# ywz978020607/MASIC

Hardware: AMD Instinct MI355X
Metric: stereo pairs/sec (enc+dec) (higher is better)
Workload: dtype bf16; 1 GPU; HSIC(N=128,M=192,K=5) eval forward (enc+dec both views), 8x3x512x512 stereo pairs per GPU (BASELINE.json configs[1] shape), inputs resident in HBM (the graph's static input buffers); the device homography of batch k+1 is handed over with batch k (one-batch look-ahead of a loader): its device->host read, the float32 host chain and the upload of the sampling matrices are done every step, under the r; pairs_per_gpu=8, height=512, width=512, parallelism=dp1 (pairs sharded, no data-path collective)

## Files before the change

masic_amd/csrc/conv.hip:

```cpp
#include "common.h"
#include "conv_geom.h"

namespace {
struct ConvCfg {
    int direct;
    int wvm;
    int wm;
    int wn;
    int buf_sz;
    int vec4;
    int bf16;
    int pf;
    int KC, KClog;
    int TW, TWlog, SR, TH;
    int Cin_pad, Cout_pad;
    int PH, PW, PWp, PSZ;
    int max_taps;
    size_t lds_bytes;
};

int ilog2(int v) { int l = 0; while ((1 << l) < v) ++l; return l; }

ConvCfg choose_cfg(const masic_conv_desc_t& d, const ConvGeom* g, int nphase) {
    ConvCfg c{};
// ... 537 lines not shown
            st.y = apply_act(acc[ph][1][o] + bv, a.act);
            *reinterpret_cast<float2*>(yo + (size_t)(2 * r + ph) * a.Wo + 2 * c) = st;
        }
    }
}

__global__ void pack_deconv4_kernel(const float* __restrict__ w, float* __restrict__ wp, int Cin, int Cin_pad, int Cout) {
    const int i = blockIdx.x * blockDim.x + threadIdx.x;
    if (i >= Cin_pad * 100) return;
    const int ci = i / 100, rem = i - ci * 100, tap = rem >> 2, o = rem & 3;
    wp[i] = (ci < Cin && o < Cout) ? w[((size_t)ci * Cout + o) * 25 + tap] : 0.0f;
}


typedef __bf16 bf16x8 __attribute__((ext_vector_type(8)));
constexpr int MAXP = 6;

__device__ __forceinline__ unsigned pack_bf16x2(float lo, float hi) {
    typedef __bf16 bf16x2 __attribute__((ext_vector_type(2)));
    bf16x2 v;
    v[0] = (__bf16)lo;
    v[1] = (__bf16)hi;
    return __builtin_bit_cast(unsigned, v);
}

template <int WVM, int WM, int WN, int INOP, bool PF>
__global__ __launch_bounds__(256, 2) void conv_igemm_bf16(const IgemmArgs a, const unsigned short* __restrict__ wpk) {
    constexpr int BM = 32 * WM * WVM;
    constexpr int DEPTH = WM * WN >= 8 ? 4 : (WM * WN >= 2 ? 8 : 16);
    extern __shared__ __attribute__((aligned(16))) float lds[];
    unsigned short* patch = reinterpret_cast<unsigned short*>(lds);
    const int KCP = a.KC + 8;
    const int tid = threadIdx.x, lane = tid & 63;
    const int wave = __builtin_amdgcn_readfirstlane(tid >> 6);
    const int wm = wave % WVM, wn = wave / WVM;
    const int j = lane & 31, h = lane >> 5;

    const int phase = blockIdx.x % a.nphase, tile = blockIdx.x / a.nphase;
    const ConvGeom g = make_geom(a.q, phase);
    const int tw_i = tile % a.tiles_w, th_i = tile / a.tiles_w;
    const int m0 = blockIdx.y * BM;
    const int b = blockIdx.z;
    const int r0 = th_i * a.TH, c0 = tw_i * a.TW;
    const int ih0 = r0 * g.is + g.dh_min, iw0 = c0 * g.is + g.dw_min;

    const int NP = a.PH * a.PW;
    const size_t plane = (size_t)a.Hi * a.Wi;
    const float* xb = a.x + ((size_t)b * a.in_ctot + a.in_coff) * plane;
    auto pixel_offset = [&](int p) {
        const int pr = p / a.PW, pc = p - pr * a.PW;
        const int ih = ih0 + pr, iw = iw0 + pc;
        return (ih >= 0 && ih < a.Hi && iw >= 0 && iw < a.Wi) ? ih * a.Wi + iw : -1;
    };
    constexpr int NT = PF ? 4 : MAXP;
    int goff[NT], gch_t[PF ? 4 : 1], loff[PF ? 4 : 1];
    const int ngroups = a.KC >> 3;
#pragma unroll
    for (int i = 0; i < NT; ++i) {
        const int t = tid + 256 * i;
        if (PF) {
            const int gq = t / NP, p = t - gq * NP;
            goff[i] = gq >= ngroups ? -2 : pixel_offset(p);
            gch_t[i] = gq * 8;
            loff[i] = p * KCP + gq * 8;
        } else {
            goff[i] = t >= NP ? -2 : pixel_offset(t);
        }
    }

    const int jr = j >> a.TWlog, jc = j & (a.TW - 1);
    int lane_p[WN];
#pragma unroll
    for (int n = 0; n < WN; ++n) {
        const int r = (wn * WN + n) * a.SR + jr;
        lane_p[n] = ((r * g.is) * a.PW + jc * g.is) * KCP + 8 * h;
    }
    f32x16 acc[WM][WN];
#pragma unroll
    for (int m = 0; m < WM; ++m)
#pragma unroll
        for (int n = 0; n < WN; ++n)
#pragma unroll
            for (int e = 0; e < 16; ++e) acc[m][n][e] = 0.0f;

    const int ksteps = a.KC >> 4, kslog = ksteps >> 1;
    const int nsteps = g.ntaps * ksteps;
    const int tap0_off = ((g.dh0 - g.dh_min) * a.PW + (g.dw0 - g.dw_min)) * KCP;
    const int row_step = (g.dsh * a.PW - g.dsw * (g.ntw - 1)) * KCP;
    const int col_step = g.dsw * KCP;
    const int cin16 = a.Cin_pad >> 4;
    const size_t a_lane = ((size_t)m0 + wm * (32 * WM) + j) * 16 + 8 * h;
    const size_t a_tap_stride = (size_t)cin16 * a.Cout_pad * 16;
    const size_t a_c16_stride = (size_t)a.Cout_pad * 16;

    float pre[PF ? 4 : 1][8];
    auto load_tasks = [&](int cc) {
#pragma unroll
        for (int i = 0; i < (PF ? 4 : 1); ++i) {
#pragma unroll
            for (int c = 0; c < 8; ++c) {
                const int cg = cc + gch_t[i] + c;
                pre[i][c] = xb[(size_t)(cg < a.Cin ? cg : a.Cin - 1) * plane + (goff[i] >= 0 ? goff[i] : 0)];
            }
        }
    };
    auto store_tasks = [&](int cc) {
#pragma unroll
        for (int i = 0; i < (PF ? 4 : 1); ++i) {
            if (goff[i] == -2) continue;
            float v[8];
#pragma unroll
            for (int c = 0; c < 8; ++c)
                v[c] = (goff[i] >= 0 && cc + gch_t[i] + c < a.Cin) ? apply_inop(pre[i][c], INOP) : 0.0f;
            uint4 q;
            q.x = pack_bf16x2(v[0], v[1]); q.y = pack_bf16x2(v[2], v[3]);
            q.z = pack_bf16x2(v[4], v[5]); q.w = pack_bf16x2(v[6], v[7]);
            *reinterpret_cast<uint4*>(patch + loff[i]) = q;
        }
    };
    if (PF) load_tasks(0);

    for (int cc = 0; cc < a.Cin_pad; cc += a.KC) {
        if (PF) {
            store_tasks(cc);
        } else {
            for (int gch = 0; gch < a.KC; gch += 8) {
                float v[NT][8];
#pragma unroll
                for (int c = 0; c < 8; ++c) {
                    const int cg = cc + gch + c;
                    if (cg < a.Cin) {
                        const float* xc = xb + (size_t)cg * plane;
#pragma unroll
                        for (int i = 0; i < NT; ++i) {
                            const float t = xc[goff[i] >= 0 ? goff[i] : 0];
                            v[i][c] = goff[i] >= 0 ? t : 0.0f;
                        }
                    } else {
#pragma unroll
                        for (int i = 0; i < NT; ++i) v[i][c] = 0.0f;
                    }
                }
#pragma unroll
                for (int i = 0; i < NT; ++i) {
                    if (goff[i] == -2) continue;
                    uint4 q;
                    q.x = pack_bf16x2(apply_inop(v[i][0], INOP), apply_inop(v[i][1], INOP));
                    q.y = pack_bf16x2(apply_inop(v[i][2], INOP), apply_inop(v[i][3], INOP));
                    q.z = pack_bf16x2(apply_inop(v[i][4], INOP), apply_inop(v[i][5], INOP));
                    q.w = pack_bf16x2(apply_inop(v[i][6], INOP), apply_inop(v[i][7], INOP));
                    *reinterpret_cast<uint4*>(patch + (size_t)(tid + 256 * i) * KCP + gch) = q;
                }
            }
        }
        __syncthreads();
        if (PF && cc + a.KC < a.Cin_pad) load_tasks(cc + a.KC);
        const unsigned short* wa = wpk + (size_t)g.tap_base * a_tap_stride + (size_t)(cc >> 4) * a_c16_stride + a_lane;
        auto a_offset = [&](int st) { return (size_t)(st >> kslog) * a_tap_stride + (size_t)(st & (ksteps - 1)) * a_c16_stride; };
        uint4 ring[DEPTH][WM];
#pragma unroll
        for (int u = 0; u < DEPTH; ++u)
            if (u < nsteps) {
                const unsigned short* pa = wa + a_offset(u);
#pragma unroll
                for (int m = 0; m < WM; ++m) ring[u][m] = *reinterpret_cast<const uint4*>(pa + m * 32 * 16);
            }
        int sp = tap0_off, kk = 0, tb = 0;
        for (int st0 = 0; st0 < nsteps; st0 += DEPTH) {
#pragma unroll
            for (int u = 0; u < DEPTH; ++u) {
                const int st = st0 + u;
                if (st < nsteps) {
                    bf16x8 bfrag[WN], afr[WM];
#pragma unroll
                    for (int n = 0; n < WN; ++n)
                        bfrag[n] = __builtin_bit_cast(bf16x8, *reinterpret_cast<const uint4*>(patch + sp + lane_p[n] + kk * 16));
#pragma unroll
                    for (int m = 0; m < WM; ++m) afr[m] = __builtin_bit_cast(bf16x8, ring[u][m]);
                    if (st + DEPTH < nsteps) {
                        const unsigned short* pa = wa + a_offset(st + DEPTH);
#pragma unroll
                        for (int m = 0; m < WM; ++m) ring[u][m] = *reinterpret_cast<const uint4*>(pa + m * 32 * 16);
                    }
#pragma unroll
                    for (int m = 0; m < WM; ++m)
#pragma unroll
                        for (int n = 0; n < WN; ++n)
                            acc[m][n] = __builtin_amdgcn_mfma_f32_32x32x16_bf16(afr[m], bfrag[n], acc[m][n], 0, 0, 0);
                    if (++kk == ksteps) {
                        kk = 0;
                        if (++tb < g.ntw) sp += col_step;
                        else { tb = 0; sp += row_step; }
                    }
                }
            }
        }
        __syncthreads();
    }

    if (a.y16 != nullptr) {
        igemm_epilogue_f16k<WM, WN>(a, g, acc, b, m0 + wm * (32 * WM), r0, c0, wn, jr, jc, h);
        return;
    }
    igemm_epilogue<WM, WN>(a, g, acc, b, m0 + wm * (32 * WM), r0, c0, wn, jr, jc, h);
}


struct Conv5s1Args {
    const float* x; const float* bias; const float* gate; const float* res1; float* y;
    int Cin, H, W, in_ctot, in_coff, Cout, out_ctot, out_coff, act, tiles_w, gate_ctot, gate_c;
    const float* xb;
    int split;
    const float* gin_beta; const float* gin_gamma; int gin_inverse;
    const float* gout_beta; const float* gout_gamma; int gout_inverse;
    float beta_bound, gamma_bound, pedestal;
};

__device__ __forceinline__ void gdn3(float (&v)[3], const float* beta, const float* gamma, int inverse, float bb, float gb, float ped) {
    float sq[3], o[3];
#pragma unroll
    for (int k = 0; k < 3; ++k) sq[k] = __fmul_rn(v[k], v[k]);
#pragma unroll
    for (int i = 0; i < 3; ++i) {
        const float bv = fmaxf(beta[i], bb);
        float n = __fsub_rn(__fmul_rn(bv, bv), ped);
        float s = 0.0f;
#pragma unroll
        for (int k = 0; k < 3; ++k) {
            const float g = fmaxf(gamma[i * 3 + k], gb);
            s = fmaf(__fsub_rn(__fmul_rn(g, g), ped), sq[k], s);
        }
        n += s;
        const float r = sqrtf(n);
        o[i] = inverse ? v[i] * r : v[i] * (1.0f / r);
    }
#pragma unroll
    for (int i = 0; i < 3; ++i) v[i] = o[i];
}

template <int CO>
__global__ __launch_bounds__(256) void conv5s1_small(const Conv5s1Args a, const float* __restrict__ wpk) {
    constexpr int T = 16, LW = T + 4, PLANE = LW * LW, PSZ = 448;
    __shared__ __attribute__((aligned(16))) float lds[8 * PSZ];
    const int tid = threadIdx.x, lane = tid & 63;
    const int wave = __builtin_amdgcn_readfirstlane(tid >> 6);
    const int tx = tid & 15, ty = ((tid >> 4) & 3) * 4 + (tid >> 6);
    const int tile_x = blockIdx.x % a.tiles_w, tile_y = blockIdx.x / a.tiles_w;
    const int b = blockIdx.y;
    const int oy = tile_y * T + ty, ox = tile_x * T + tx;
    const size_t plane = (size_t)a.H * a.W;
    const float* xb = a.x + ((size_t)b * a.in_ctot + a.in_coff) * plane;
    const int split = a.xb != nullptr ? a.split : a.Cin;
    const float* xb2 = a.xb != nullptr ? a.xb + (size_t)b * (a.Cin - split) * plane : nullptr;
    for (int cg = wave; cg < a.Cin * 7; cg += 4) {
        const int ci = cg / 7, g = cg - ci * 7;
        const int e = g * 64 + lane;
        const int pr = e / LW, pc = e - pr * LW;
        const int ih = tile_y * T - 2 + pr, iw = tile_x * T - 2 + pc;
        const bool ok = e < PLANE && ih >= 0 && ih < a.H && iw >= 0 && iw < a.W;
        const float* src = ci < split ? xb + (size_t)ci * plane : xb2 + (size_t)(ci - split) * plane;
        if (e < PLANE) dma4(ok ? src + (size_t)ih * a.W + iw : g_zero_word, lds + ci * PSZ + g * 64);
    }
    __syncthreads();
    if (a.gin_beta != nullptr) {
        for (int e = tid; e < PLANE; e += 256) {
            float v[3] = {lds[e], lds[PSZ + e], lds[2 * PSZ + e]};
            gdn3(v, a.gin_beta, a.gin_gamma, a.gin_inverse, a.beta_bound, a.gamma_bound, a.pedestal);
            lds[e] = v[0]; lds[PSZ + e] = v[1]; lds[2 * PSZ + e] = v[2];
        }
        __syncthreads();
    }
    float acc[CO];
#pragma unroll
    for (int o = 0; o < CO; ++o) acc[o] = 0.0f;
    const float* base = lds + ty * LW + tx;
    for (int ci = 0; ci < a.Cin; ++ci) {
        const float* w = wpk + ci * 25 * CO;
        const float* pl = base + ci * PSZ;
#pragma unroll
        for (int kh = 0; kh < 5; ++kh)
#pragma unroll
            for (int kw = 0; kw < 5; ++kw) {
                const float xv = pl[kh * LW + kw];
#pragma unroll
                for (int o = 0; o < CO; ++o) acc[o] = fmaf(xv, w[(kh * 5 + kw) * CO + o], acc[o]);
            }
    }
    if (oy >= a.H || ox >= a.W) return;
    const size_t opix = (size_t)oy * a.W + ox;
    const float gv = a.gate ? a.gate[((size_t)b * a.gate_ctot + a.gate_c) * plane + opix] : 1.0f;
    if (a.gout_beta != nullptr) {
        float v[3] = {acc[0] + (a.bias ? a.bias[0] : 0.0f), acc[1] + (a.bias ? a.bias[1] : 0.0f), acc[2] + (a.bias ? a.bias[2] : 0.0f)};
        gdn3(v, a.gout_beta, a.gout_gamma, a.gout_inverse, a.beta_bound, a.gamma_bound, a.pedestal);
#pragma unroll
        for (int o = 0; o < 3; ++o) a.y[((size_t)b * a.out_ctot + a.out_coff + o) * plane + opix] = v[o];
        return;
    }
#pragma unroll
    for (int o = 0; o < CO; ++o) {
        if (o >= a.Cout) break;
        float v = apply_act(acc[o] + (a.bias ? a.bias[o] : 0.0f), a.act) * gv;
        if (a.res1) v += a.res1[((size_t)b * a.Cout + o) * plane + opix];
        a.y[((size_t)b * a.out_ctot + a.out_coff + o) * plane + opix] = v;
    }
}

__global__ void pack_conv5s1_kernel(const float* __restrict__ w, float* __restrict__ wp, int Cin, int Cout, int transposed, int CO) {
    const int i = blockIdx.x * blockDim.x + threadIdx.x;
    if (i >= Cin * 25 * CO) return;
    const int ci = i / (25 * CO), rem = i - ci * 25 * CO, tap = rem / CO, o = rem - tap * CO;
    float v = 0.0f;
    if (o < Cout) v = transposed ? w[((size_t)ci * Cout + o) * 25 + (24 - tap)] : w[((size_t)o * Cin + ci) * 25 + tap];
    wp[i] = v;
}


}

extern "C" size_t masic_conv_packed_bytes(const masic_conv_desc_t* d) {
    if (check_desc(d) != MASIC_OK) return 0;
    ConvGeom g[4];
    const int np = build_geoms(*d, g);
    const ConvCfg c = choose_cfg(*d, g, np);
    int taps = 0;
    for (int p = 0; p < np; ++p) taps += g[p].ntaps;
    if (c.direct == 2) return (size_t)c.Cin_pad * 100 * sizeof(float);
    if (c.direct == 3) return (size_t)c.Cin_pad * 25 * c.Cout_pad * sizeof(float);
    if (c.bf16) return (size_t)taps * c.Cin_pad * c.Cout_pad * sizeof(unsigned short);
    return (size_t)taps * c.Cin_pad * c.Cout_pad * sizeof(float);
}

extern "C" int masic_conv_variant(const masic_conv_desc_t* d, int* launches) {
    int rc = check_desc(d);
    if (rc != MASIC_OK) return rc;
    ConvGeom g[4];
    const int np = build_geoms(*d, g);
    const ConvCfg c = choose_cfg(*d, g, np);
    if (launches) *launches = 1;
    if (c.direct == 2) return 6;
    if (c.direct == 3) return 11;
    if (c.direct) return d->Cout <= 3 ? 0 : 1;
    if (c.bf16) return 10;
    if (c.wvm == 1) return c.wm == 1 ? 8 : 9;
    if (c.wm == 2) return c.wn == 4 ? 5 : 7;
    return c.wn == 4 ? 4 : (c.wn == 2 ? 3 : 2);
}

extern "C" int masic_conv_kernel_name(const masic_conv_desc_t* d, char* buf, size_t n) {
    int rc = check_desc(d);
    if (rc != MASIC_OK) return rc;
    MASIC_REQUIRE(buf && n > 0, MASIC_ERR_ARG, "conv_kernel_name: null buffer");
    ConvGeom g[4];
    const int np = build_geoms(*d, g);
    const ConvCfg c = choose_cfg(*d, g, np);
    if (c.direct == 2) snprintf(buf, n, "deconv5s2_small_cout");
    else if (c.direct == 3) snprintf(buf, n, "conv5s1_small");
    else if (c.direct) snprintf(buf, n, "conv_direct_f32<%d>", d->Cout <= 3 ? 3 : 8);
    else if (c.bf16) snprintf(buf, n, "conv_igemm_bf16<%d, %d, %d, %d, %s>", c.wvm, c.wm, c.wn, d->in_op, c.pf ? "true" : "false");
    else snprintf(buf, n, "conv_igemm_f32<%d, %d, %d, %d, %s>", c.wvm, c.wm, c.wn, d->in_op, c.vec4 ? "true" : "false");
    return MASIC_OK;
}

extern "C" int masic_conv_pack_weight(const float* w, void* w_packed, const masic_conv_desc_t* d, void* stream) {
    int rc = check_desc(d);
    if (rc != MASIC_OK) return rc;
    MASIC_REQUIRE(w && w_packed, MASIC_ERR_ARG, "conv_pack_weight: null pointer");
    ConvGeom g[4];
    const int np = build_geoms(*d, g);
    const ConvCfg c = choose_cfg(*d, g, np);
    if (c.direct == 2) {
        hipLaunchKernelGGL(pack_deconv4_kernel, dim3(ceil_div(c.Cin_pad * 100, 256)), dim3(256), 0, (hipStream_t)stream,
                           w, (float*)w_packed, d->Cin, c.Cin_pad, d->Cout);
        return masic_launch_status("conv_pack_weight");
    }
    if (c.direct == 3) {
        hipLaunchKernelGGL(pack_conv5s1_kernel, dim3(ceil_div(d->Cin * 25 * c.Cout_pad, 256)), dim3(256), 0, (hipStream_t)stream,
                           w, (float*)w_packed, d->Cin, d->Cout, d->transposed, c.Cout_pad);
        return masic_launch_status("conv_pack_weight");
    }
    PackArgs a{w, (float*)w_packed, d->Cin, d->Cout, d->KH, d->KW, c.Cin_pad, c.Cout_pad, d->transposed, {}};
    int max_taps = 0;
    for (int p = 0; p < np; ++p) {
        a.gs[p] = g[p];
        max_taps = max_taps > g[p].ntaps ? max_taps : g[p].ntaps;
    }
    const size_t total = (size_t)max_taps * c.Cin_pad * c.Cout_pad;
    int blocks = (int)((total + 255) / 256);
    if (blocks > 4096) blocks = 4096;
    if (c.bf16) hipLaunchKernelGGL(pack_weight_bf16_kernel, dim3(blocks, np), dim3(256), 0, (hipStream_t)stream, a, (unsigned short*)w_packed);
    else hipLaunchKernelGGL(pack_weight_kernel, dim3(blocks, np), dim3(256), 0, (hipStream_t)stream, a);
    return masic_launch_status("conv_pack_weight");
}

extern "C" int masic_conv2d_fwd_ex(const float* x, const void* w_packed, const float* bias, const float* gate,
                                   const float* res1, const float* res2, float* y, const masic_conv_desc_t* d, void* stream);

extern "C" int masic_conv2d_fwd(const float* x, const void* w_packed, const float* bias, const float* gate,
                                float* y, const masic_conv_desc_t* d, void* stream) {
    return masic_conv2d_fwd_ex(x, w_packed, bias, gate, nullptr, nullptr, y, d, stream);
}

namespace {
int conv2d_launch(const float* x, const void* w_packed, const float* bias, const float* gate,
                  const float* res1, const float* res2, float* y, void* y_f16k, const masic_conv_desc_t* d, void* stream);
}

extern "C" int masic_conv2d_fwd_ex(const float* x, const void* w_packed, const float* bias, const float* gate,
                                   const float* res1, const float* res2, float* y, const masic_conv_desc_t* d, void* stream) {
    MASIC_REQUIRE(y != nullptr, MASIC_ERR_ARG, "conv2d_fwd: null pointer");
    return conv2d_launch(x, w_packed, bias, gate, res1, res2, y, nullptr, d, stream);
}

extern "C" int masic_conv2d_f16k_out_supported(const masic_conv_desc_t* d) {
    if (check_desc(d) != MASIC_OK || d->prec != MASIC_PREC_BF16 || d->Cout % 32 != 0 || d->out_ctot % 16 != 0 || d->out_coff % 16 != 0) return 0;
    ConvGeom g[4];
    const int np = build_geoms(*d, g);
    const ConvCfg c = choose_cfg(*d, g, np);
    return !c.direct && c.bf16;
}

extern "C" int masic_conv2d_f16k_out_fwd(const float* x, const void* w_packed, const float* bias, void* y_f16k,
                                         const masic_conv_desc_t* d, void* stream) {
    MASIC_REQUIRE(y_f16k != nullptr && d != nullptr, MASIC_ERR_ARG, "conv2d_f16k_out_fwd: null pointer");
    MASIC_REQUIRE(masic_conv2d_f16k_out_supported(d), MASIC_ERR_UNSUPPORTED,
                  "conv2d_f16k_out_fwd: needs bf16 operands on the implicit-GEMM kernel, Cout % 32 == 0 and a 16-aligned output view");
    return conv2d_launch(x, w_packed, bias, nullptr, nullptr, nullptr, nullptr, y_f16k, d, stream);
}

namespace {
int conv2d_launch(const float* x, const void* w_packed, const float* bias, const float* gate,
                  const float* res1, const float* res2, float* y, void* y_f16k, const masic_conv_desc_t* d, void* stream) {
    int rc = check_desc(d);
    if (rc != MASIC_OK) return rc;
    MASIC_REQUIRE(d->prec != MASIC_PREC_FP8, MASIC_ERR_UNSUPPORTED, "conv2d_fwd: fp8 operands exist on the F8K entry points only (masic_conv_f8k_fwd)");
    MASIC_REQUIRE(x && w_packed && (y || y_f16k), MASIC_ERR_ARG, "conv2d_fwd: null pointer");
    ConvGeom g[4];
    const int np = build_geoms(*d, g);
    const ConvCfg c = choose_cfg(*d, g, np);
    MASIC_REQUIRE(y_f16k == nullptr || (!c.direct && c.bf16), MASIC_ERR_UNSUPPORTED, "conv2d_fwd: F16K output exists on conv_igemm_bf16 only");
    hipStream_t st = (hipStream_t)stream;
    const GeomParams q = geom_params(*d);
    if (g[0].Hp <= 0 || g[0].Wp <= 0) return MASIC_OK;
    if (c.direct == 2) {
        MASIC_REQUIRE(gate == nullptr && res1 == nullptr && res2 == nullptr, MASIC_ERR_UNSUPPORTED, "conv2d_fwd: gate/residual on the small-Cout deconv path");
        MASIC_REQUIRE(d->Wo % 2 == 0, MASIC_ERR_SHAPE, "conv2d_fwd: odd output width");
        Deconv4Args a{x, (const float*)w_packed, bias, y, d->Cin, c.Cin_pad, d->Hi, d->Wi, d->in_ctot, d->in_coff,
                      d->Cout, d->Ho, d->Wo, d->out_ctot, d->out_coff, d->act, ceil_div(d->Wi, 16)};
        hipLaunchKernelGGL(deconv5s2_small_cout, dim3(ceil_div(d->Wi, 16) * ceil_div(d->Hi, 16), d->B), dim3(256), 0, st, a,
                           (const float*)w_packed);
        return masic_launch_status("conv2d_fwd");
    }
    if (c.direct == 3) {
        MASIC_REQUIRE(res2 == nullptr, MASIC_ERR_UNSUPPORTED, "conv2d_fwd: two residuals on the small 5x5 path");
        Conv5s1Args a{x, bias, gate, res1, y, d->Cin, d->Hi, d->Wi, d->in_ctot, d->in_coff, d->Cout, d->out_ctot, d->out_coff,
                      d->act, ceil_div(d->Wi, 16), d->gate_ctot, d->gate_c, nullptr, 0, nullptr, nullptr, 0, nullptr, nullptr, 0, 0.0f, 0.0f, 0.0f};
        if (c.Cout_pad == 4) hipLaunchKernelGGL(conv5s1_small<4>, dim3(ceil_div(d->Wi, 16) * ceil_div(d->Hi, 16), d->B), dim3(256), 0, st, a,
                                                (const float*)w_packed);
        else hipLaunchKernelGGL(conv5s1_small<8>, dim3(ceil_div(d->Wi, 16) * ceil_div(d->Hi, 16), d->B), dim3(256), 0, st, a,
                                (const float*)w_packed);
        return masic_launch_status("conv2d_fwd");
    }
    if (c.direct) {
        DirectArgs a{x, (const float*)w_packed, bias, gate, res1, res2, y,
                     d->Cin, d->Hi, d->Wi, d->in_ctot, d->in_coff,
                     d->Cout, d->Ho, d->Wo, d->out_ctot, d->out_coff,
                     d->in_op, d->act, d->gate_ctot, d->gate_c, q, np};
        dim3 grid(ceil_div(g[0].Hp * g[0].Wp, 256) * np, d->B);
        if (d->Cout <= 3) hipLaunchKernelGGL(conv_direct_f32<3>, grid, dim3(256), 0, st, a);
        else hipLaunchKernelGGL(conv_direct_f32<8>, grid, dim3(256), 0, st, a);
        return masic_launch_status("conv2d_fwd");
    }
    {
        IgemmArgs a{x, (const float*)w_packed, bias, gate, res1, res2, y,
                    d->Cin, d->Hi, d->Wi, d->in_ctot, d->in_coff,
                    d->Cout, d->Ho, d->Wo, d->out_ctot, d->out_coff,
                    c.Cin_pad, c.Cout_pad, c.KC, c.KClog,
                    c.TW, c.TWlog, c.SR, c.TH, ceil_div(g[0].Wp, c.TW),
                    c.PH, c.PW, c.PWp, c.PSZ, c.buf_sz, c.vec4,
                    d->in_op, d->act, d->gate_ctot, d->gate_c, q, np, (unsigned short*)y_f16k};
        dim3 grid(ceil_div(g[0].Wp, c.TW) * ceil_div(g[0].Hp, c.TH) * np, c.Cout_pad / (32 * c.wm * c.wvm), d->B);
        if (c.bf16) {
#define BF16_LAUNCH(WV, WMV, WNV, OPV)                                                                                            \
    do {                                                                                                                          \
        if (c.pf) hipLaunchKernelGGL((conv_igemm_bf16<WV, WMV, WNV, OPV, true>), grid, dim3(256), c.lds_bytes, st, a,             \
                                     (const unsigned short*)w_packed);                                                           \
        else hipLaunchKernelGGL((conv_igemm_bf16<WV, WMV, WNV, OPV, false>), grid, dim3(256), c.lds_bytes, st, a,                 \
                                (const unsigned short*)w_packed);                                                                 \
    } while (0)
#define BF16_BY_OP(WV, WMV, WNV)                                                       \
    do {                                                                               \
        if (d->in_op == MASIC_INOP_ABS) BF16_LAUNCH(WV, WMV, WNV, MASIC_INOP_ABS);     \
        else if (d->in_op == MASIC_INOP_ROUND) BF16_LAUNCH(WV, WMV, WNV, MASIC_INOP_ROUND); \
        else BF16_LAUNCH(WV, WMV, WNV, MASIC_INOP_NONE);                               \
    } while (0)
            if (c.wvm == 1 && c.wm == 1) BF16_BY_OP(1, 1, 2);
            else if (c.wvm == 1) BF16_BY_OP(1, 3, 2);
            else if (c.wm == 2 && c.wn == 4) BF16_BY_OP(2, 2, 4);
            else if (c.wm == 2 && c.wn == 2) BF16_BY_OP(2, 2, 2);
            else if (c.wm == 2) BF16_BY_OP(2, 2, 1);
            else if (c.wn == 4) BF16_BY_OP(2, 1, 4);
            else if (c.wn == 2) BF16_BY_OP(2, 1, 2);
            else BF16_BY_OP(2, 1, 1);
#undef BF16_BY_OP
#undef BF16_LAUNCH
            return masic_launch_status("conv2d_fwd");
        }
#define IGEMM_LAUNCH(WV, WMV, WNV, OPV, V4) \
    hipLaunchKernelGGL((conv_igemm_f32<WV, WMV, WNV, OPV, V4>), grid, dim3(256), c.lds_bytes, st, a)
#define IGEMM_BY_OP(WV, WMV, WNV)                                                               \
    do {                                                                                        \
        if (d->in_op == MASIC_INOP_ABS) IGEMM_LAUNCH(WV, WMV, WNV, MASIC_INOP_ABS, false);      \
        else if (d->in_op == MASIC_INOP_ROUND) IGEMM_LAUNCH(WV, WMV, WNV, MASIC_INOP_ROUND, false); \
        else if (c.vec4) IGEMM_LAUNCH(WV, WMV, WNV, MASIC_INOP_NONE, true);                     \
        else IGEMM_LAUNCH(WV, WMV, WNV, MASIC_INOP_NONE, false);                                \
    } while (0)
        if (c.wvm == 1 && c.wm == 1) IGEMM_BY_OP(1, 1, 2);
        else if (c.wvm == 1) IGEMM_BY_OP(1, 3, 2);
        else if (c.wm == 2 && c.wn == 4) IGEMM_BY_OP(2, 2, 4);
        else if (c.wm == 2) IGEMM_BY_OP(2, 2, 2);
        else if (c.wn == 4) IGEMM_BY_OP(2, 1, 4);
        else if (c.wn == 2) IGEMM_BY_OP(2, 1, 2);
        else IGEMM_BY_OP(2, 1, 1);
#undef IGEMM_BY_OP
#undef IGEMM_LAUNCH
    }
    return masic_launch_status("conv2d_fwd");
}
}

extern "C" int masic_conv5s1_pair_fwd(const float* xa, const float* xb, const float* w_packed, const float* bias,
                                      const float* gin_beta, const float* gin_gamma, int gin_inverse,
                                      const float* gout_beta, const float* gout_gamma, int gout_inverse, double beta_min,
                                      float* y, int B, int H, int W, void* stream) {
    MASIC_REQUIRE(xa && xb && w_packed && y, MASIC_ERR_ARG, "conv5s1_pair_fwd: null pointer");
    MASIC_REQUIRE(B > 0 && H > 0 && W > 0, MASIC_ERR_SHAPE, "conv5s1_pair_fwd: non-positive dimension");
    MASIC_REQUIRE((gin_beta == nullptr) == (gin_gamma == nullptr) && (gout_beta == nullptr) == (gout_gamma == nullptr), MASIC_ERR_ARG,
                  "conv5s1_pair_fwd: a GDN needs both beta and gamma");
    const double ped = 0x1p-36;
    Conv5s1Args a{xa, bias, nullptr, nullptr, y, 6, H, W, 3, 0, 3, 3, 0, MASIC_ACT_NONE, ceil_div(W, 16), 0, 0,
                  xb, 3, gin_beta, gin_gamma, gin_inverse, gout_beta, gout_gamma, gout_inverse,
                  (float)__builtin_sqrt(beta_min + ped), (float)__builtin_sqrt(ped), (float)ped};
    hipLaunchKernelGGL(conv5s1_small<4>, dim3(ceil_div(W, 16) * ceil_div(H, 16), B), dim3(256), 0, (hipStream_t)stream, a, (const float*)w_packed);
    return masic_launch_status("conv5s1_pair_fwd");
}
```

Measured before the change: 4096 stereo pairs/s.

## Add dedicated 32x32-tile pair conv kernel with 4-pixel register blocking

Replaces the generic conv5s1_small<4> launch for the 6-to-3 channel stereo pair 5x5 conv with a specialised kernel. It uses 32x32 output tiles staged in LDS, with each thread computing 4 horizontal pixels times 3 outputs from a sliding 8-float register window, and writes results with float4 stores. The aim is more reuse per LDS read and fewer blocks, lowering LDS and halo overhead. The trade-offs are more LDS per block, fewer blocks for small images, and a new code path that must match the old numerics for the GDN in/out fusion.

```diff
diff --git a/masic_amd/csrc/conv.hip b/masic_amd/csrc/conv.hip
--- a/masic_amd/csrc/conv.hip
+++ b/masic_amd/csrc/conv.hip
@@ -863,6 +863,86 @@
         float v = apply_act(acc[o] + (a.bias ? a.bias[o] : 0.0f), a.act) * gv;
         if (a.res1) v += a.res1[((size_t)b * a.Cout + o) * plane + opix];
         a.y[((size_t)b * a.out_ctot + a.out_coff + o) * plane + opix] = v;
+    }
+}
+
+__global__ __launch_bounds__(256) void conv5s1_pair3(const Conv5s1Args a, const float* __restrict__ wpk) {
+    constexpr int T = 32, LW = T + 4, PLANE = LW * LW, NG = (PLANE + 63) / 64, PSZ = NG * 64, CIN = 6;
+    __shared__ __attribute__((aligned(16))) float lds[CIN * PSZ];
+    const int tid = threadIdx.x, lane = tid & 63;
+    const int wave = __builtin_amdgcn_readfirstlane(tid >> 6);
+    const int tx = lane & 7, ty = ((lane >> 3) & 3) * 8 + (lane >> 5) + 2 * wave;
+    const int tile_x = blockIdx.x % a.tiles_w, tile_y = blockIdx.x / a.tiles_w;
+    const int b = blockIdx.y;
+    const size_t plane = (size_t)a.H * a.W;
+    const float* xa = a.x + ((size_t)b * a.in_ctot + a.in_coff) * plane;
+    const float* xb2 = a.xb + (size_t)b * (CIN - a.split) * plane;
+    for (int g = wave; g < NG; g += 4) {
+        const int e = g * 64 + lane;
+        const int pr = e / LW, pc = e - pr * LW;
+        const int ih = tile_y * T - 2 + pr, iw = tile_x * T - 2 + pc;
+        const bool ok = e < PLANE && ih >= 0 && ih < a.H && iw >= 0 && iw < a.W;
+        const size_t off = ok ? (size_t)ih * a.W + iw : 0;
+        if (e < PLANE) {
+#pragma unroll
+            for (int ci = 0; ci < CIN; ++ci) {
+                const float* src = ci < a.split ? xa + (size_t)ci * plane : xb2 + (size_t)(ci - a.split) * plane;
+                dma4(ok ? src + off : g_zero_word, lds + ci * PSZ + g * 64);
+            }
+        }
+    }
+    __syncthreads();
+    if (a.gin_beta != nullptr) {
+        for (int e = tid; e < PLANE; e += 256) {
+            float v[3] = {lds[e], lds[PSZ + e], lds[2 * PSZ + e]};
+            gdn3(v, a.gin_beta, a.gin_gamma, a.gin_inverse, a.beta_bound, a.gamma_bound, a.pedestal);
+            lds[e] = v[0]; lds[PSZ + e] = v[1]; lds[2 * PSZ + e] = v[2];
+        }
+        __syncthreads();
+    }
+    float acc[4][3];
+#pragma unroll
+    for (int p = 0; p < 4; ++p)
+#pragma unroll
+        for (int o = 0; o < 3; ++o) acc[p][o] = 0.0f;
+    const float* base = lds + ty * LW + 4 * tx;
+#pragma unroll 1
+    for (int ci = 0; ci < CIN; ++ci) {
+        const float* w = wpk + ci * 100;
+        const float* pl = base + ci * PSZ;
+#pragma unroll
+        for (int kh = 0; kh < 5; ++kh) {
+            const float4 lo = *reinterpret_cast<const float4*>(pl + kh * LW);
+            const float4 hi = *reinterpret_cast<const float4*>(pl + kh * LW + 4);
+            const float xv[8] = {lo.x, lo.y, lo.z, lo.w, hi.x, hi.y, hi.z, hi.w};
+#pragma unroll
+            for (int kw = 0; kw < 5; ++kw)
+#pragma unroll
+                for (int p = 0; p < 4; ++p)
+#pragma unroll
+                    for (int o = 0; o < 3; ++o) acc[p][o] = fmaf(xv[p + kw], w[(kh * 5 + kw) * 4 + o], acc[p][o]);
+        }
+    }
+    const int oy = tile_y * T + ty, ox = tile_x * T + 4 * tx;
+    if (oy >= a.H || ox >= a.W) return;
+    float out[3][4];
+#pragma unroll
+    for (int p = 0; p < 4; ++p) {
+        float v[3] = {acc[p][0] + (a.bias ? a.bias[0] : 0.0f), acc[p][1] + (a.bias ? a.bias[1] : 0.0f), acc[p][2] + (a.bias ? a.bias[2] : 0.0f)};
+        if (a.gout_beta != nullptr) gdn3(v, a.gout_beta, a.gout_gamma, a.gout_inverse, a.beta_bound, a.gamma_bound, a.pedestal);
+#pragma unroll
+        for (int o = 0; o < 3; ++o) out[o][p] = v[o];
+    }
+    const bool vec = (a.W & 3) == 0 && (reinterpret_cast<size_t>(a.y) & 15) == 0;
+#pragma unroll
+    for (int o = 0; o < 3; ++o) {
+        float* yp = a.y + ((size_t)b * a.out_ctot + a.out_coff + o) * plane + (size_t)oy * a.W + ox;
+        if (vec) *reinterpret_cast<float4*>(yp) = make_float4(out[o][0], out[o][1], out[o][2], out[o][3]);
+        else {
+#pragma unroll
+            for (int p = 0; p < 4; ++p)
+                if (ox + p < a.W) yp[p] = out[o][p];
+        }
     }
 }
 
@@ -1098,9 +1178,9 @@
     MASIC_REQUIRE((gin_beta == nullptr) == (gin_gamma == nullptr) && (gout_beta == nullptr) == (gout_gamma == nullptr), MASIC_ERR_ARG,
                   "conv5s1_pair_fwd: a GDN needs both beta and gamma");
     const double ped = 0x1p-36;
-    Conv5s1Args a{xa, bias, nullptr, nullptr, y, 6, H, W, 3, 0, 3, 3, 0, MASIC_ACT_NONE, ceil_div(W, 16), 0, 0,
+    Conv5s1Args a{xa, bias, nullptr, nullptr, y, 6, H, W, 3, 0, 3, 3, 0, MASIC_ACT_NONE, ceil_div(W, 32), 0, 0,
                   xb, 3, gin_beta, gin_gamma, gin_inverse, gout_beta, gout_gamma, gout_inverse,
                   (float)__builtin_sqrt(beta_min + ped), (float)__builtin_sqrt(ped), (float)ped};
-    hipLaunchKernelGGL(conv5s1_small<4>, dim3(ceil_div(W, 16) * ceil_div(H, 16), B), dim3(256), 0, (hipStream_t)stream, a, (const float*)w_packed);
+    hipLaunchKernelGGL(conv5s1_pair3, dim3(ceil_div(W, 32) * ceil_div(H, 32), B), dim3(256), 0, (hipStream_t)stream, a, (const float*)w_packed);
     return masic_launch_status("conv5s1_pair_fwd");
 }
```

After: 4114 stereo pairs/s, median of 6. Within noise of the previous version (+0.4%).

## Add row-tiled 5x5 pair conv kernel with buffer-to-LDS loads and vector outputs

Applied to the files above, without the earlier changes.

Adds a specialized kernel for the 6-in/3-out stereo pair 5x5 conv. Each thread computes four horizontal outputs from a shared register window, and 64x16 tiles are staged into LDS with direct buffer-load-to-LDS instructions. The input GDN is applied in LDS and the three output channels are written as float4 stores. It runs only when widths and pointers are 16-byte aligned and the plane fits a buffer offset, otherwise it falls back to the old kernel. The aim is to reduce LDS reads and global load overhead per output, at the cost of more registers and more padded halo per tile.

```diff
diff --git a/masic_amd/csrc/conv.hip b/masic_amd/csrc/conv.hip
--- a/masic_amd/csrc/conv.hip
+++ b/masic_amd/csrc/conv.hip
@@ -864,6 +864,93 @@
         if (a.res1) v += a.res1[((size_t)b * a.Cout + o) * plane + opix];
         a.y[((size_t)b * a.out_ctot + a.out_coff + o) * plane + opix] = v;
     }
+}
+
+typedef float f32x2 __attribute__((ext_vector_type(2)));
+typedef float f32x4 __attribute__((ext_vector_type(4)));
+
+__global__ __launch_bounds__(256, 4) void conv5s1_pair_rows(const Conv5s1Args a, const float* __restrict__ wpk) {
+    constexpr int TW = 64, TH = 16, LP = TW + 8, LR = TH + 4, RP = LP / 4, PCS = LR * RP, PSZ = 6 * 256;
+    constexpr int OOR = 0x7ffffff0;
+    __shared__ __attribute__((aligned(16))) float lds[6 * PSZ];
+    const int tid = threadIdx.x, lane = tid & 63;
+    const int wave = __builtin_amdgcn_readfirstlane(tid >> 6);
+    const int tx = tid & 15, ty = wave * 2 + ((tid >> 5) & 1) + ((tid >> 4) & 1) * 8;
+    const int tile_x = blockIdx.x % a.tiles_w, tile_y = blockIdx.x / a.tiles_w;
+    const int b = blockIdx.y;
+    const size_t plane = (size_t)a.H * a.W;
+    const float* srca = a.x + (size_t)b * 3 * plane;
+    const float* srcb = a.xb + (size_t)b * 3 * plane;
+#pragma unroll
+    for (int k = 0; k < 9; ++k) {
+        const int cg = k * 4 + wave;
+        const int ci = cg / 6, g = cg - ci * 6;
+        const int e = g * 64 + lane;
+        const int pr = e / RP, pc = e - pr * RP;
+        const int ih = tile_y * TH - 2 + pr, iw = tile_x * TW - 4 + pc * 4;
+        const bool ok = e < PCS && ih >= 0 && ih < a.H && iw >= 0 && iw < a.W;
+        const __amdgpu_buffer_rsrc_t r = __builtin_amdgcn_make_buffer_rsrc((void*)(ci < 3 ? srca : srcb), 0, (int)(3 * plane * 4), 0x00020000);
+        const int c3 = ci < 3 ? ci : ci - 3;
+        __builtin_amdgcn_raw_ptr_buffer_load_lds(r, (__attribute__((address_space(3))) void*)(lds + cg * 256), 16,
+                                                 ok ? ((c3 * a.H + ih) * a.W + iw) * 4 : OOR, 0, 0, 0);
+    }
+    __syncthreads();
+    if (a.gin_beta != nullptr) {
+        for (int e = tid; e < PCS; e += 256) {
+            f32x4 p[3];
+#pragma unroll
+            for (int c = 0; c < 3; ++c) p[c] = *reinterpret_cast<const f32x4*>(lds + c * PSZ + e * 4);
+#pragma unroll
+            for (int j = 0; j < 4; ++j) {
+                float v[3] = {p[0][j], p[1][j], p[2][j]};
+                gdn3(v, a.gin_beta, a.gin_gamma, a.gin_inverse, a.beta_bound, a.gamma_bound, a.pedestal);
+                p[0][j] = v[0]; p[1][j] = v[1]; p[2][j] = v[2];
+            }
+#pragma unroll
+            for (int c = 0; c < 3; ++c) *reinterpret_cast<f32x4*>(lds + c * PSZ + e * 4) = p[c];
+        }
+        __syncthreads();
+    }
+    f32x2 acc01[4];
+    float acc2[4];
+#pragma unroll
+    for (int j = 0; j < 4; ++j) { acc01[j] = f32x2{0.0f, 0.0f}; acc2[j] = 0.0f; }
+    const float* base = lds + ty * LP + tx * 4;
+    for (int ci = 0; ci < 6; ++ci) {
+        const float* w = wpk + ci * 100;
+        const float* pl = base + ci * PSZ;
+#pragma unroll
+        for (int kh = 0; kh < 5; ++kh) {
+            f32x4 lo = *reinterpret_cast<const f32x4*>(pl + kh * LP);
+            const f32x4 mid = *reinterpret_cast<const f32x4*>(pl + kh * LP + 4);
+            f32x4 hi = *reinterpret_cast<const f32x4*>(pl + kh * LP + 8);
+            asm("" : "+v"(lo), "+v"(hi));
+            const float win[8] = {lo[2], lo[3], mid[0], mid[1], mid[2], mid[3], hi[0], hi[1]};
+#pragma unroll
+            for (int kw = 0; kw < 5; ++kw) {
+                const f32x2 w01 = *reinterpret_cast<const f32x2*>(w + (kh * 5 + kw) * 4);
+                const float w2 = w[(kh * 5 + kw) * 4 + 2];
+#pragma unroll
+                for (int j = 0; j < 4; ++j) {
+                    const float xv = win[j + kw];
+                    acc01[j] = __builtin_elementwise_fma(f32x2{xv, xv}, w01, acc01[j]);
+                    acc2[j] = fmaf(xv, w2, acc2[j]);
+                }
+            }
+        }
+    }
+    const int oy = tile_y * TH + ty, ox = tile_x * TW + tx * 4;
+    if (oy >= a.H || ox >= a.W) return;
+    f32x4 out[3];
+#pragma unroll
+    for (int j = 0; j < 4; ++j) {
+        float v[3] = {acc01[j][0] + (a.bias ? a.bias[0] : 0.0f), acc01[j][1] + (a.bias ? a.bias[1] : 0.0f), acc2[j] + (a.bias ? a.bias[2] : 0.0f)};
+        if (a.gout_beta != nullptr) gdn3(v, a.gout_beta, a.gout_gamma, a.gout_inverse, a.beta_bound, a.gamma_bound, a.pedestal);
+        out[0][j] = v[0]; out[1][j] = v[1]; out[2][j] = v[2];
+    }
+    float* yb = a.y + (size_t)b * 3 * plane + (size_t)oy * a.W + ox;
+#pragma unroll
+    for (int o = 0; o < 3; ++o) *reinterpret_cast<f32x4*>(yb + (size_t)o * plane) = out[o];
 }
 
 __global__ void pack_conv5s1_kernel(const float* __restrict__ w, float* __restrict__ wp, int Cin, int Cout, int transposed, int CO) {
@@ -1101,6 +1188,13 @@
     Conv5s1Args a{xa, bias, nullptr, nullptr, y, 6, H, W, 3, 0, 3, 3, 0, MASIC_ACT_NONE, ceil_div(W, 16), 0, 0,
                   xb, 3, gin_beta, gin_gamma, gin_inverse, gout_beta, gout_gamma, gout_inverse,
                   (float)__builtin_sqrt(beta_min + ped), (float)__builtin_sqrt(ped), (float)ped};
-    hipLaunchKernelGGL(conv5s1_small<4>, dim3(ceil_div(W, 16) * ceil_div(H, 16), B), dim3(256), 0, (hipStream_t)stream, a, (const float*)w_packed);
+    const bool rows = W % 4 == 0 && (((uintptr_t)xa | (uintptr_t)xb | (uintptr_t)w_packed | (uintptr_t)y) & 15) == 0 &&
+                      (size_t)3 * H * W * 4 <= (size_t)0x7ffffff0;
+    if (rows) {
+        a.tiles_w = ceil_div(W, 64);
+        hipLaunchKernelGGL(conv5s1_pair_rows, dim3(ceil_div(W, 64) * ceil_div(H, 16), B), dim3(256), 0, (hipStream_t)stream, a, (const float*)w_packed);
+    } else {
+        hipLaunchKernelGGL(conv5s1_small<4>, dim3(ceil_div(W, 16) * ceil_div(H, 16), B), dim3(256), 0, (hipStream_t)stream, a, (const float*)w_packed);
+    }
     return masic_launch_status("conv5s1_pair_fwd");
 }
```

After: 4157 stereo pairs/s before, 4217 stereo pairs/s after (median of 6 runs). 1.4% higher.
